# mkkellogg/GaussianSplats3D

Measured on NVIDIA H100. Metric: frames_per_sec, higher is better.
Workload: dtype int32 sort keys / f32 raster

## Files before the change

gaussiansplats3d_b200/csrc/raster_kernels.cuh:

```cuda
#pragma once
#include "common.cuh"
#include "sort_kernels.cuh"
#include "../../include/gsplat_b200.h"
#include <cuda_fp16.h>
#include "ellipse_mask.h"

namespace gs {

constexpr int kTile = 16;
constexpr int kTileShift = 4;
constexpr float kTransmittanceCutoff = 1.0f / 512.0f;

struct __align__(16) SplatRecord {
    float cx, cy;
    float g1x, g1y;
    float g2x, g2y;
    uint32_t hxhy;
    float a;
    float r, g, b;
    float ndc_z;
};

constexpr int kVisibleSlots = 64;
struct RasterControl {
// ... 83 lines not shown
        for (int r = 0; r < 4; ++r)
            o[4 * c + r] = a[r] * b[4 * c] + a[4 + r] * b[4 * c + 1] + a[8 + r] * b[4 * c + 2] + a[12 + r] * b[4 * c + 3];
}
__device__ inline void mat4_inverse_dev(const float *m, float *o) {
    float inv[16];
    inv[0] = m[5] * m[10] * m[15] - m[5] * m[11] * m[14] - m[9] * m[6] * m[15] + m[9] * m[7] * m[14] + m[13] * m[6] * m[11] - m[13] * m[7] * m[10];
    inv[4] = -m[4] * m[10] * m[15] + m[4] * m[11] * m[14] + m[8] * m[6] * m[15] - m[8] * m[7] * m[14] - m[12] * m[6] * m[11] + m[12] * m[7] * m[10];
    inv[8] = m[4] * m[9] * m[15] - m[4] * m[11] * m[13] - m[8] * m[5] * m[15] + m[8] * m[7] * m[13] + m[12] * m[5] * m[11] - m[12] * m[7] * m[9];
    inv[12] = -m[4] * m[9] * m[14] + m[4] * m[10] * m[13] + m[8] * m[5] * m[14] - m[8] * m[6] * m[13] - m[12] * m[5] * m[10] + m[12] * m[6] * m[9];
    inv[1] = -m[1] * m[10] * m[15] + m[1] * m[11] * m[14] + m[9] * m[2] * m[15] - m[9] * m[3] * m[14] - m[13] * m[2] * m[11] + m[13] * m[3] * m[10];
    inv[5] = m[0] * m[10] * m[15] - m[0] * m[11] * m[14] - m[8] * m[2] * m[15] + m[8] * m[3] * m[14] + m[12] * m[2] * m[11] - m[12] * m[3] * m[10];
    inv[9] = -m[0] * m[9] * m[15] + m[0] * m[11] * m[13] + m[8] * m[1] * m[15] - m[8] * m[3] * m[13] - m[12] * m[1] * m[11] + m[12] * m[3] * m[9];
    inv[13] = m[0] * m[9] * m[14] - m[0] * m[10] * m[13] - m[8] * m[1] * m[14] + m[8] * m[2] * m[13] + m[12] * m[1] * m[10] - m[12] * m[2] * m[9];
    inv[2] = m[1] * m[6] * m[15] - m[1] * m[7] * m[14] - m[5] * m[2] * m[15] + m[5] * m[3] * m[14] + m[13] * m[2] * m[7] - m[13] * m[3] * m[6];
    inv[6] = -m[0] * m[6] * m[15] + m[0] * m[7] * m[14] + m[4] * m[2] * m[15] - m[4] * m[3] * m[14] - m[12] * m[2] * m[7] + m[12] * m[3] * m[6];
    inv[10] = m[0] * m[5] * m[15] - m[0] * m[7] * m[13] - m[4] * m[1] * m[15] + m[4] * m[3] * m[13] + m[12] * m[1] * m[7] - m[12] * m[3] * m[5];
    inv[14] = -m[0] * m[5] * m[14] + m[0] * m[6] * m[13] + m[4] * m[1] * m[14] - m[4] * m[2] * m[13] - m[12] * m[1] * m[6] + m[12] * m[2] * m[5];
    inv[3] = -m[1] * m[6] * m[11] + m[1] * m[7] * m[10] + m[5] * m[2] * m[11] - m[5] * m[3] * m[10] - m[9] * m[2] * m[7] + m[9] * m[3] * m[6];
    inv[7] = m[0] * m[6] * m[11] - m[0] * m[7] * m[10] - m[4] * m[2] * m[11] + m[4] * m[3] * m[10] + m[8] * m[2] * m[7] - m[8] * m[3] * m[6];
    inv[11] = -m[0] * m[5] * m[11] + m[0] * m[7] * m[9] + m[4] * m[1] * m[11] - m[4] * m[3] * m[9] - m[8] * m[1] * m[7] + m[8] * m[3] * m[5];
    inv[15] = m[0] * m[5] * m[10] - m[0] * m[6] * m[9] - m[4] * m[1] * m[10] + m[4] * m[2] * m[9] + m[8] * m[1] * m[6] - m[8] * m[2] * m[5];
    const float det = m[0] * inv[0] + m[1] * inv[4] + m[2] * inv[8] + m[3] * inv[12];
    const float id = 1.0f / det;
#pragma unroll
    for (int i = 0; i < 16; ++i) o[i] = inv[i] * id;
}

constexpr int kProjThreads = 128;

template <bool COVF16, int SHFMT>
__global__ void __launch_bounds__(kProjThreads)
k_project(const uint4 *__restrict__ cc, const void *__restrict__ cov, const void *__restrict__ sh, int sh_data_degree,
          const uint32_t *__restrict__ scene_idx, const DynamicUniforms *__restrict__ dyn, const ProjParams *__restrict__ Pp, uint32_t count,
          SplatRecord *__restrict__ rec, ushort4 *__restrict__ rects, RasterControl *rctl) {
    pdl_enter();
    __shared__ ProjParams s_P;
    {
        const uint32_t *src = reinterpret_cast<const uint32_t *>(Pp);
        uint32_t *dst = reinterpret_cast<uint32_t *>(&s_P);
        for (int i = threadIdx.x; i < (int)(sizeof(ProjParams) / 4); i += kProjThreads) dst[i] = __ldg(src + i);
    }
    __syncthreads();
    const ProjParams &P = s_P;
    __shared__ float4 s_out[kProjThreads / 32][96];
    const uint32_t lane = threadIdx.x & 31;
    const uint32_t s = blockIdx.x * kProjThreads + threadIdx.x;
    uint32_t visible = 0;
    if (s < count) {
        SplatRecord o;
        o.cx = o.cy = o.g1x = o.g1y = o.g2x = o.g2y = o.a = o.r = o.g = o.b = 0.f;
        o.ndc_z = 2.0f;
        o.hxhy = 0;
        ushort4 rect = make_ushort4(1, 1, 0, 0);
        const int4 c4 = ld_nc_v4(cc + s);
        float V[6];
        if (COVF16) {
            const uint32_t *h32 = (const uint32_t *)cov + (size_t)s * 3;
#pragma unroll
            for (int k = 0; k < 3; ++k) {
                const uint32_t w = ld_nc_u32(h32 + k);
                const __half2 hh = *reinterpret_cast<const __half2 *>(&w);
                V[2 * k] = __low2float(hh); V[2 * k + 1] = __high2float(hh);
            }
        } else {
            const float2 *f2 = (const float2 *)cov + (size_t)s * 3;
            const float2 a0 = __ldg(f2), a1 = __ldg(f2 + 1), a2 = __ldg(f2 + 2);
            V[0] = a0.x; V[1] = a0.y; V[2] = a1.x; V[3] = a1.y; V[4] = a2.x; V[5] = a2.y;
// ... 139 lines not shown
                o.cy = (ndcy + 1.0f) * 0.5f * P.viewport[1];
                o.g1x = ex * is1; o.g1y = ey * is1;
                o.g2x = ey * is2; o.g2y = -ex * is2;
                o.ndc_z = ndcz; o.a = col[3];
                o.r = col[0]; o.g = col[1]; o.b = col[2];
                const bool in_depth = (ndcz >= -1.0f && ndcz <= 1.0f) && isfinite(s1) && isfinite(s2) && s1 > 0.f && s2 > 0.f;
                if (!in_depth && ndcz >= -1.0f && ndcz <= 1.0f) o.ndc_z = 2.0f;
                if (in_depth) {
                    const float b1x = ex * s1, b1y = ey * s1, b2x = ey * s2, b2y = -ex * s2;
                    const float hx = sqrtf(b1x * b1x + b2x * b2x) * 1.0005f + 0.01f;
                    const float hy = sqrtf(b1y * b1y + b2y * b2y) * 1.0005f + 0.01f;
                    const __half2 hh = __halves2half2(__float2half_ru(fminf(hx, 60000.f)), __float2half_ru(fminf(hy, 60000.f)));
                    o.hxhy = *reinterpret_cast<const uint32_t *>(&hh);
                    const float fx0 = ceilf(o.cx - hx - 0.5f), fx1 = floorf(o.cx + hx - 0.5f);
                    const float fy0 = ceilf(o.cy - hy - 0.5f), fy1 = floorf(o.cy + hy - 0.5f);
                    const float W1 = (float)(P.width - 1), H1 = (float)(P.height - 1);
                    if (fx1 >= 0.f && fy1 >= 0.f && fx0 <= W1 && fy0 <= H1 && fx0 <= fx1 && fy0 <= fy1) {
                        const int px0 = (int)fmaxf(fx0, 0.f), px1 = (int)fminf(fx1, W1);
                        const int py0 = (int)fmaxf(fy0, 0.f), py1 = (int)fminf(fy1, H1);
                        rect = make_ushort4((unsigned short)(px0 >> P.tile_shift), (unsigned short)(py0 >> P.tile_shift),
                                            (unsigned short)(px1 >> P.tile_shift), (unsigned short)(py1 >> P.tile_shift));
                        visible = 1;
                    }
                }
            }
        }
        float4 *stage = s_out[threadIdx.x >> 5];
        stage[lane * 3 + 0] = make_float4(o.cx, o.cy, o.g1x, o.g1y);
        stage[lane * 3 + 1] = make_float4(o.g2x, o.g2y, __uint_as_float(o.hxhy), o.a);
        stage[lane * 3 + 2] = make_float4(o.r, o.g, o.b, o.ndc_z);
        rects[s] = rect;
    }
    __syncwarp();
    {
        const uint32_t warp_first = blockIdx.x * kProjThreads + (threadIdx.x & ~31u);
        if (warp_first < count) {
            const uint32_t nrec = min(32u, count - warp_first);
            float4 *gdst = reinterpret_cast<float4 *>(rec + warp_first);
            const float4 *stage = s_out[threadIdx.x >> 5];
#pragma unroll
            for (int k = 0; k < 3; ++k) {
                const uint32_t idx = (uint32_t)k * 32 + lane;
                if (idx < nrec * 3) gdst[idx] = stage[idx];
            }
        }
    }
    const uint32_t nvis = __popc(__ballot_sync(0xffffffffu, visible));
    if ((threadIdx.x & 31) == 0 && nvis) atomicAdd(&rctl->visible_slots[((blockIdx.x * (kProjThreads / 32) + (threadIdx.x >> 5)) & (kVisibleSlots - 1)) * 8], nvis);
}

constexpr int kCoarseW = 8, kCoarseH = 4, kCoarseShiftX = 3, kCoarseShiftY = 2;
constexpr int kFinePerCoarse = kCoarseW * kCoarseH;

struct OwnMask { unsigned long long lo, hi; };
__host__ __device__ __forceinline__ bool own_diag(const OwnMask &m, int diag) {
    return ((diag < 64 ? m.lo >> diag : m.hi >> (diag - 64)) & 1ull) != 0ull;
}
__device__ __forceinline__ uint32_t own_count_range(const OwnMask &m, int d0, int d1) {
    uint32_t n = 0;
    if (d0 < 64) {
        const int hi = min(d1, 63);
        const unsigned long long w = (m.lo >> d0) & (hi - d0 == 63 ? ~0ull : ((1ull << (hi - d0 + 1)) - 1ull));
        n += __popcll(w);
    }
    if (d1 >= 64) {
        const int lo = max(d0, 64) - 64, hi = d1 - 64;
        const unsigned long long w = (m.hi >> lo) & (hi - lo == 63 ? ~0ull : ((1ull << (hi - lo + 1)) - 1ull));
        n += __popcll(w);
    }
    return n;
}
static inline OwnMask make_own_mask(uint32_t rank, uint32_t world) {
    OwnMask m{~0ull, ~0ull};
    if (world > 1) {
        m.lo = m.hi = 0;
        for (int d = 0; d < 128; ++d)
            if ((uint32_t)d % world == rank) { if (d < 64) m.lo |= 1ull << d; else m.hi |= 1ull << (d - 64); }
    }
    return m;
}
// ... 173 lines not shown

template <typename F>
__device__ __forceinline__ void round_instances(bool valid, uint32_t sid, ushort4 r, int coarse_x, const OwnMask &own, bool sharded, F f) {
    const int lane = threadIdx.x & 31;
    const bool nonempty = valid && r.z >= r.x && r.w >= r.y;
    const int cx0 = r.x >> kCoarseShiftX, cx1 = r.z >> kCoarseShiftX, cy0 = r.y >> kCoarseShiftY, cy1 = r.w >> kCoarseShiftY;
    const bool big = nonempty && (uint32_t)(cx1 - cx0 + 1) * (uint32_t)(cy1 - cy0 + 1) > 32u;
    if (nonempty && !big) {
#pragma unroll 1
        for (int cy = cy0; cy <= cy1; ++cy)
#pragma unroll 1
            for (int cx = cx0; cx <= cx1; ++cx) {
                if (sharded && !own_diag(own, cx + cy)) continue;
                f(lane, sid, cy * coarse_x + cx, fine_mask_in_coarse((int)r.x, (int)r.y, (int)r.z, (int)r.w, cx, cy));
            }
    }
    uint32_t multi = __ballot_sync(0xffffffffu, big);
    while (multi) {
        const int src = __ffs(multi) - 1;
        multi &= multi - 1;
        const uint32_t bsid = __shfl_sync(0xffffffffu, sid, src);
        const int bx0 = __shfl_sync(0xffffffffu, (int)r.x, src), by0 = __shfl_sync(0xffffffffu, (int)r.y, src);
        const int bx1 = __shfl_sync(0xffffffffu, (int)r.z, src), by1 = __shfl_sync(0xffffffffu, (int)r.w, src);
        const int ccx0 = bx0 >> kCoarseShiftX, ccy0 = by0 >> kCoarseShiftY;
        const int cw = (bx1 >> kCoarseShiftX) - ccx0 + 1, ntile = cw * ((by1 >> kCoarseShiftY) - ccy0 + 1);
        for (int i = lane; i < ntile; i += 32) {
            const int cy = ccy0 + i / cw, cx = ccx0 + i % cw;
            if (sharded && !own_diag(own, cx + cy)) continue;
            f(src, bsid, cy * coarse_x + cx, fine_mask_in_coarse(bx0, by0, bx1, by1, cx, cy));
        }
    }
}

__global__ void __launch_bounds__(kBinWarps * 32)
k_bin_count(const uint32_t *__restrict__ order, uint32_t render_count_host, const unsigned long long *__restrict__ n_dev, const ushort4 *__restrict__ rects,
            int coarse_x, uint32_t nt, uint32_t *__restrict__ hist, uint32_t stride, uint32_t *__restrict__ totals, ushort4 *__restrict__ rect_by_rank,
            OwnMask own, int sharded) {
    pdl_enter();
    constexpr int W = kBinWarps, ITEMS = kBinRankItems, NT = kBinTiles;
    const uint32_t n = n_dev ? (uint32_t)*n_dev : render_count_host;
    const uint32_t base = blockIdx.x * (uint32_t)(W * 32 * ITEMS);
    if (base >= n) return;
    __shared__ uint32_t s_hist[NT];
    for (uint32_t t = threadIdx.x; t < nt; t += W * 32) s_hist[t] = 0;
    __syncthreads();
    const int lane = threadIdx.x & 31, warp = threadIdx.x >> 5;
    const uint32_t run = base + (uint32_t)warp * (32 * ITEMS) + lane;
    uint32_t sid[ITEMS];
    ushort4 rc[ITEMS];
#pragma unroll
    for (int k = 0; k < ITEMS; ++k) {
        const uint32_t p = run + (uint32_t)k * 32;
        sid[k] = p < n ? ld_nc_u32(order + (n - 1u - p)) : 0xffffffffu;
    }
#pragma unroll
    for (int k = 0; k < ITEMS; ++k) rc[k] = sid[k] != 0xffffffffu ? rects[sid[k]] : make_ushort4(1, 1, 0, 0);
#pragma unroll
    for (int k = 0; k < ITEMS; ++k) {
        const uint32_t p = run + (uint32_t)k * 32;
        if (p < n) rect_by_rank[p] = rc[k];
    }
#pragma unroll 1
    for (int k = 0; k < ITEMS; ++k) {
        uint32_t id = 0; ushort4 r = make_ushort4(1, 1, 0, 0);
#pragma unroll
        for (int j = 0; j < ITEMS; ++j) if (j == k) { id = sid[j]; r = rc[j]; }
        round_instances(id != 0xffffffffu, id, r, coarse_x, own, sharded != 0, [&](int, uint32_t, int t, uint32_t) { atomicAdd(&s_hist[t], 1u); });
    }
    __syncthreads();
    for (uint32_t t = threadIdx.x; t < nt; t += W * 32) {
        const uint32_t v = s_hist[t];
        hist[(size_t)t * stride + blockIdx.x] = v;
        if (v) atomicAdd(&totals[t], v);
    }
}

__global__ void __launch_bounds__(1024)
k_bin_scan(uint32_t *__restrict__ hist, uint32_t stride, uint32_t ranks_per_chunk, uint32_t render_count_host, const unsigned long long *__restrict__ n_dev,
           const uint32_t *__restrict__ totals, uint32_t nt, uint2 *__restrict__ ranges, RasterControl *rctl, uint32_t *__restrict__ tile_order,
           unsigned long long capacity) {
    pdl_enter();
    __shared__ uint32_t s_scan[40];
    __shared__ uint32_t s_carry;
    {
        const uint32_t mine = totals[blockIdx.x];
        bool ahead = false;
        if (threadIdx.x < nt) { const uint32_t o = totals[threadIdx.x]; ahead = o > mine || (o == mine && threadIdx.x < blockIdx.x); }
        const int rank = __syncthreads_count(ahead);
        if (threadIdx.x == 0) tile_order[rank] = blockIdx.x;
    }
    const uint32_t n = n_dev ? (uint32_t)*n_dev : render_count_host;
    const uint32_t nchunks = (uint32_t)(((uint64_t)n + ranks_per_chunk - 1) / ranks_per_chunk);
    const uint32_t d = blockIdx.x;
    {
        uint32_t total;
        const uint32_t c = threadIdx.x < d ? totals[threadIdx.x] : 0u;
        (void)block_exclusive_scan<1024>(c, s_scan, total);
        if (threadIdx.x == 0) {
            s_carry = total;
            const uint32_t mine = totals[d];
            const unsigned long long lo = total, hi = lo + mine;
            ranges[d] = make_uint2((uint32_t)min(lo, capacity), (uint32_t)min(hi, capacity));
            if (d == nt - 1) rctl->total_instances = hi;
        }
    }
    __syncthreads();
    uint32_t *col = hist + (size_t)d * stride;
    for (uint32_t b = 0; b < nchunks; b += 1024) {
        const uint32_t t = b + threadIdx.x;
        const uint32_t v = t < nchunks ? col[t] : 0u;
        uint32_t total;
        const uint32_t ex = block_exclusive_scan<1024>(v, s_scan, total);
        const uint32_t carry = s_carry;
        if (t < nchunks) col[t] = ex + carry;
        __syncthreads();
        if (threadIdx.x == 0) s_carry = carry + total;
        __syncthreads();
    }
}

__global__ void __launch_bounds__(kBinWarps * 32)
k_bin_place(const uint32_t *__restrict__ order, uint32_t render_count_host, const unsigned long long *__restrict__ n_dev, const ushort4 *__restrict__ rect_by_rank,
            int coarse_x, uint32_t nt, const uint32_t *__restrict__ offsets, uint32_t stride, unsigned long long *__restrict__ list, unsigned long long capacity,
            RasterControl *rctl, OwnMask own, int sharded, int pack_ok) {
    pdl_enter();
    constexpr int W = kBinWarps, ITEMS = kBinRankItems, NT = kBinTiles;
    const uint32_t n = n_dev ? (uint32_t)*n_dev : render_count_host;
    const uint32_t base = blockIdx.x * (uint32_t)(W * 32 * ITEMS);
    if (base >= n) return;
    __shared__ uint32_t s_pre[W][NT];
    __shared__ __align__(8) uint32_t s_mask[W][NT];
    static_assert(NT * 4 >= 32 * ITEMS * 8, "the mask row of a warp doubles as the staging buffer of its compacted items");
    for (uint32_t i = threadIdx.x; i < (uint32_t)(W * NT); i += W * 32) (&s_pre[0][0])[i] = 0;
    __syncthreads();
    const int lane = threadIdx.x & 31, warp = threadIdx.x >> 5;
    const uint32_t run = base + (uint32_t)warp * (32 * ITEMS) + lane;
    uint32_t sid[ITEMS];
    ushort4 rc[ITEMS];
#pragma unroll
    for (int k = 0; k < ITEMS; ++k) {
        const uint32_t p = run + (uint32_t)k * 32;
        sid[k] = p < n ? ld_nc_u32(order + (n - 1u - p)) : 0xffffffffu;
        rc[k] = p < n ? rect_by_rank[p] : make_ushort4(1, 1, 0, 0);
    }
    uint32_t *my_pre = s_pre[warp], *my_mask = s_mask[warp];
    uint32_t nvalid = 32u * ITEMS;
    if (pack_ok) {
        const uint32_t lt = lanemask_lt();
        unsigned long long *stage = reinterpret_cast<unsigned long long *>(my_mask);
        uint32_t before = 0;
#pragma unroll
        for (int k = 0; k < ITEMS; ++k) {
            const bool keep = sid[k] != 0xffffffffu && (sharded ? rect_touches_owned(rc[k], own) : (rc[k].z >= rc[k].x && rc[k].w >= rc[k].y));
            const uint32_t bal = __ballot_sync(0xffffffffu, keep);
            if (keep) stage[before + __popc(bal & lt)] = ((unsigned long long)((uint32_t)rc[k].x | ((uint32_t)rc[k].y << 8) | ((uint32_t)rc[k].z << 16) | ((uint32_t)rc[k].w << 24)) << 32) | sid[k];
            before += __popc(bal);
        }
        nvalid = before;
        __syncwarp();
#pragma unroll
        for (int k = 0; k < ITEMS; ++k) {
            const uint32_t j = (uint32_t)k * 32u + (uint32_t)lane;
            sid[k] = 0xffffffffu;
            rc[k] = make_ushort4(1, 1, 0, 0);
            if (j < nvalid) {
                const unsigned long long v = stage[j];
                const uint32_t pr = (uint32_t)(v >> 32);
                sid[k] = (uint32_t)v;
                rc[k] = make_ushort4((unsigned short)(pr & 255u), (unsigned short)((pr >> 8) & 255u), (unsigned short)((pr >> 16) & 255u), (unsigned short)(pr >> 24));
            }
        }
        __syncwarp();
#pragma unroll
        for (int i = 0; i < NT / 32; ++i) my_mask[i * 32 + lane] = 0u;
        __syncwarp();
    }
#pragma unroll
    for (int k = 0; k < ITEMS; ++k)
        if ((uint32_t)k * 32u < nvalid)
            round_instances(sid[k] != 0xffffffffu, sid[k], rc[k], coarse_x, own, sharded != 0, [&](int, uint32_t, int t, uint32_t) { atomicAdd(&my_pre[t], 1u); });
    __syncthreads();
    for (uint32_t t = threadIdx.x; t < nt; t += W * 32) {
        uint32_t at = offsets[(size_t)t * stride + blockIdx.x];
#pragma unroll
        for (int w = 0; w < W; ++w) {
            const uint32_t c = s_pre[w][t];
            s_pre[w][t] = at;
            at += c;
        }
    }
    __syncthreads();
    bool overflow = false;
#pragma unroll
    for (int k = 0; k < ITEMS; ++k) {
        if ((uint32_t)k * 32u >= nvalid) break;
        const bool valid = sid[k] != 0xffffffffu;
#pragma unroll
        for (int i = 0; i < NT / 32; ++i) my_mask[i * 32 + lane] = 0u;
        __syncwarp();
        round_instances(valid, sid[k], rc[k], coarse_x, own, sharded != 0, [&](int owner, uint32_t, int t, uint32_t) {
            atomicOr(&my_mask[t], 1u << owner);
            atomicAdd(&my_pre[t], 1u);
        });
        __syncwarp();
        round_instances(valid, sid[k], rc[k], coarse_x, own, sharded != 0, [&](int owner, uint32_t sid_o, int t, uint32_t fmask) {
            const uint32_t m = my_mask[t];
            const unsigned long long at = (unsigned long long)(my_pre[t] - (uint32_t)__popc(m)) + __popc(m & ((1u << owner) - 1u));
            if (at < capacity) list[at] = ((unsigned long long)fmask << 32) | sid_o;
            else overflow = true;
        });
        __syncwarp();
    }
    if (overflow) rctl->overflow = 1;
}

__global__ void __launch_bounds__(kBinThreads)
// ... 296 lines not shown
    size_t n = 0;
    cudaError_t ensure(size_t count) {
        if (count <= n) return cudaSuccess;
        if (p) cudaFree(p);
        p = nullptr; n = 0;
        cudaError_t e = cudaMalloc((void **)&p, (count ? count : 1) * sizeof(T));
        if (e == cudaSuccess) n = count;
        return e;
    }
    void release() { if (p) cudaFree(p); p = nullptr; n = 0; }
};

struct RasterState {
    RBuf<uint4> cc;
    RBuf<unsigned char> cov, sh;
    RBuf<uint32_t> scene_idx;
    int cov_format = GS_COV_F32, sh_format = GS_SH_NONE;
    uint32_t sh_degree = 0, uploaded = 0;
    bool have_scene_idx = false;
    RBuf<SplatRecord> records;
    RBuf<ushort4> rects;
    RBuf<uint32_t> block_sums;
    RBuf<uint32_t> warp_sums;
    RBuf<uint32_t> super_sums;
    uint32_t super_stride = 0;
    RBuf<uint16_t> ikeys[2];
    RBuf<unsigned long long> ivals[2];
    RBuf<unsigned long long> list;
    RBuf<uint2> ranges;
    RBuf<RasterControl> rctl;
    RBuf<SortControl> sctl;
    RBuf<uint32_t> tile_hist;
    RBuf<uint32_t> bin_hist;
    RBuf<ushort4> rect_by_rank;
    RBuf<uint32_t> tile_order;
    RBuf<uint32_t> bin_totals;
    uint32_t bin_stride = 0;
    RBuf<DynamicUniforms> dyn;
    RBuf<ProjParams> projp;
    RBuf<unsigned char> frame;
    RBuf<unsigned char> frame_alt;
    unsigned char *frame_half2 = nullptr;
    size_t frame_half_bytes = 0;
    int frame_parity = 0;
    uint32_t *snap_base = nullptr;
    uint32_t snap_stride = 0;
    const uint32_t *snap_sort_ctl = nullptr;
    bool snapshot_taken = false;
    RBuf<gs_projected_splat> exported;
    RBuf<PeerSync> peer_sync_local;
    PeerSync *peer_sync = nullptr;
    void *peer_frame = nullptr;
    bool peer_root = false, peer_attached = false;
    unsigned long long instance_capacity = 0;
    uint32_t hist_stride = 0;
    int sm_count = 132;
    int last_format = GS_FRAME_RGBA32F;
    size_t last_frame_bytes = 0;
};

#define RCU(call)                                                                                                 \
    do {                                                                                                          \
        cudaError_t _e = (call);                                                                                  \
        if (_e != cudaSuccess) { snprintf(raster_err(), 512, "%s -> %s (%s:%d)", #call, cudaGetErrorString(_e), __FILE__, __LINE__); return GS_ERR_CUDA; } \
    } while (0)

static inline char *raster_err() { return g_gs_err; }

static inline int frame_tile_shift(uint32_t width, uint32_t height) {
    const uint32_t cx = (width + kTile * kCoarseW - 1) / (kTile * kCoarseW), cy = (height + kTile * kCoarseH - 1) / (kTile * kCoarseH);
    return (cx * cy <= (uint32_t)kBinTiles) ? kTileShift : kTileShift + 1;
}

static inline uint32_t frame_coarse_tiles(uint32_t width, uint32_t height) {
    const uint32_t tpx = 1u << frame_tile_shift(width, height);
    const uint32_t tiles_x = (width + tpx - 1) / tpx, tiles_y = (height + tpx - 1) / tpx;
    return ((tiles_x + kCoarseW - 1) / kCoarseW) * ((tiles_y + kCoarseH - 1) / kCoarseH);
}

static int raster_init(RasterState &rs, const gs_config &c, int sm_count) {
    rs.sm_count = sm_count;
    const size_t n = c.max_splat_count ? c.max_splat_count : 1;
    RCU(rs.rctl.ensure(1));
    RCU(cudaMemset(rs.rctl.p, 0, sizeof(RasterControl)));
    RCU(rs.sctl.ensure(1));
    RCU(rs.dyn.ensure(2));
    RCU(rs.projp.ensure(2));
    RCU(cudaMemset(rs.dyn.p, 0, 2 * sizeof(DynamicUniforms)));
    if (c.max_width && c.max_height) {
        RCU(rs.cc.ensure(n));
        RCU(rs.records.ensure(n));
        RCU(rs.rects.ensure(n));
        RCU(rs.block_sums.ensure((n + kBinTile - 1) / kBinTile + 1));
        RCU(rs.warp_sums.ensure(((n + kBinTile - 1) / kBinTile + 1) * (kBinThreads / 32)));
        rs.super_stride = (uint32_t)(((n + kBinTile - 1) / kBinTile) / kBinThreads + 2);
        RCU(rs.super_sums.ensure(2 * (size_t)rs.super_stride));
        const char *f = getenv("GS_INSTANCE_FACTOR");
        const double factor = f ? atof(f) : 4.0;
        const size_t tiles = (size_t)((c.max_width + kTile - 1) / kTile) * ((c.max_height + kTile - 1) / kTile);
        rs.instance_capacity = (unsigned long long)(factor * (double)n) + 4ull * tiles + 65536ull;
        if (rs.instance_capacity > 0xfffffff0ull) rs.instance_capacity = 0xfffffff0ull;
        RCU(rs.list.ensure(rs.instance_capacity));
        RCU(rs.ranges.ensure(65536));
        RCU(rs.tile_order.ensure(65536));
        RCU(rs.frame.ensure((size_t)c.max_width * (c.max_height + kTile) * 16));
        if (frame_coarse_tiles(c.max_width, c.max_height) > (uint32_t)kBinTiles) {
            for (int i = 0; i < 2; ++i) { RCU(rs.ikeys[i].ensure(rs.instance_capacity)); RCU(rs.ivals[i].ensure(rs.instance_capacity)); }
            RCU(rs.tile_hist.ensure(radix_tile_hist_words(rs.instance_capacity, 2, &rs.hist_stride)));
        }
        {
            const size_t coarse = (size_t)((c.max_width + kTile * kCoarseW - 1) / (kTile * kCoarseW)) * ((c.max_height + kTile * kCoarseH - 1) / (kTile * kCoarseH));
            const size_t chunks = (n + kBinRanks - 1) / kBinRanks + 1;
            rs.bin_stride = (uint32_t)((chunks + 31) & ~(size_t)31);
            RCU(rs.bin_hist.ensure(std::max<size_t>(coarse, 1) * rs.bin_stride));
            RCU(rs.rect_by_rank.ensure(n));
            RCU(rs.bin_totals.ensure(kBinTiles));
            RCU(cudaMemset(rs.bin_totals.p, 0, kBinTiles * 4));
        }
    }
    return GS_OK;
}

static void raster_release(RasterState &rs) {
    rs.cc.release(); rs.cov.release(); rs.sh.release(); rs.scene_idx.release(); rs.records.release(); rs.rects.release();
    rs.block_sums.release(); rs.warp_sums.release(); rs.super_sums.release(); rs.ikeys[0].release(); rs.ikeys[1].release(); rs.ivals[0].release(); rs.ivals[1].release();
    rs.list.release(); rs.ranges.release(); rs.rctl.release(); rs.sctl.release(); rs.tile_hist.release(); rs.bin_hist.release(); rs.bin_totals.release(); rs.rect_by_rank.release(); rs.tile_order.release();
    rs.dyn.release(); rs.projp.release(); rs.frame.release(); rs.frame_alt.release(); rs.peer_sync_local.release(); rs.exported.release();
}

static int raster_upload(RasterState &rs, const gs_config &c, const gs_splat_data &d, cudaStream_t st) {
    if (!c.max_width || !c.max_height) { snprintf(raster_err(), 512, "engine created without a framebuffer (max_width/max_height = 0)"); return GS_ERR_NOT_READY; }
    if ((uint64_t)d.from + d.count > c.max_splat_count) { snprintf(raster_err(), 512, "splat data [%u,%u) exceeds max_splat_count %u", d.from, d.from + d.count, c.max_splat_count); return GS_ERR_CAPACITY; }
    if (!d.centers_colors || !d.covariances) { snprintf(raster_err(), 512, "gs_upload_splat_data: null centers_colors/covariances"); return GS_ERR_BAD_ARG; }
    if (d.sh_degree > 2) { snprintf(raster_err(), 512, "sh_degree %u > 2", d.sh_degree); return GS_ERR_BAD_ARG; }
    const size_t n = c.max_splat_count;
    const size_t cov_elt = d.cov_format == GS_COV_F16 ? 12 : 24;
    const size_t ncomp = d.sh_degree == 2 ? 24 : (d.sh_degree == 1 ? 9 : 0);
    const size_t sh_elt = ncomp * (d.sh_format == GS_SH_F16 ? 2 : (d.sh_format == GS_SH_U8 ? 1 : 4));
    if (d.from == 0) rs.uploaded = 0;
    if (rs.uploaded && (rs.cov_format != d.cov_format || (rs.sh_degree != d.sh_degree) || (ncomp && rs.sh_format != d.sh_format))) {
        snprintf(raster_err(), 512, "splat data format changed between partial uploads"); return GS_ERR_BAD_ARG;
    }
    rs.cov_format = d.cov_format;
    rs.sh_degree = d.sh_degree;
    rs.sh_format = ncomp ? d.sh_format : GS_SH_NONE;
    RCU(rs.cov.ensure(n * cov_elt + 16));
    if (ncomp) {
        if (!d.spherical_harmonics) { snprintf(raster_err(), 512, "sh_degree %u without spherical_harmonics", d.sh_degree); return GS_ERR_BAD_ARG; }
        RCU(rs.sh.ensure(n * sh_elt + 16));
    }
    RCU(cudaMemcpyAsync(rs.cc.p + d.from, d.centers_colors, (size_t)d.count * 16, cudaMemcpyHostToDevice, st));
    RCU(cudaMemcpyAsync(rs.cov.p + (size_t)d.from * cov_elt, d.covariances, (size_t)d.count * cov_elt, cudaMemcpyHostToDevice, st));
    if (ncomp) RCU(cudaMemcpyAsync(rs.sh.p + (size_t)d.from * sh_elt, d.spherical_harmonics, (size_t)d.count * sh_elt, cudaMemcpyHostToDevice, st));
    if (d.scene_indexes) {
        RCU(rs.scene_idx.ensure(n));
        RCU(cudaMemcpyAsync(rs.scene_idx.p + d.from, d.scene_indexes, (size_t)d.count * 4, cudaMemcpyHostToDevice, st));
        rs.have_scene_idx = true;
    }
    rs.uploaded = std::max<uint32_t>(rs.uploaded, d.from + d.count);
    return GS_OK;
}

static unsigned char *raster_second_frame(RasterState &rs) { return rs.frame_alt.p ? rs.frame_alt.p : rs.frame_half2; }
static void *raster_frame_ptr(RasterState &rs, int) { return (rs.frame_parity && raster_second_frame(rs)) ? raster_second_frame(rs) : rs.frame.p; }

template <bool COVF16>
static void launch_project(RasterState &rs, uint32_t count, cudaStream_t st) {
    const int blocks = (int)((count + kProjThreads - 1) / kProjThreads);
    const uint32_t *sc = rs.have_scene_idx ? rs.scene_idx.p : nullptr;
#define GS_PROJ(FMT) gs_launch(k_project<COVF16, FMT>, blocks, kProjThreads, 0, st, rs.cc.p, rs.cov.p, rs.sh.p, (int)rs.sh_degree, sc, rs.dyn.p + rs.frame_parity, rs.projp.p + rs.frame_parity, count, rs.records.p, rs.rects.p, rs.rctl.p)
    switch (rs.sh_format) {
        case GS_SH_F16: GS_PROJ(GS_SH_F16); break;
        case GS_SH_U8: GS_PROJ(GS_SH_U8); break;
        case GS_SH_F32: GS_PROJ(GS_SH_F32); break;
        default: GS_PROJ(GS_SH_NONE); break;
    }
#undef GS_PROJ
}

static int raster_upload_params(RasterState &rs, const gs_config &c, const gs_uniforms &u, const gs_render_params &p, cudaStream_t st) {
    const int tshift = frame_tile_shift(p.width, p.height), tpx = 1 << tshift;
    const int tiles_x = (p.width + tpx - 1) / tpx, tiles_y = (p.height + tpx - 1) / tpx;
    const uint32_t world = c.world_size, rank = c.rank;
    ProjParams P{};
    memcpy(P.mv, u.model_view, 64); memcpy(P.proj, u.projection, 64);
    memcpy(P.cam, u.camera_position, 12);
    P.focal[0] = u.focal[0]; P.focal[1] = u.focal[1]; P.viewport[0] = u.viewport[0]; P.viewport[1] = u.viewport[1];
    P.inv_focal_adj = u.inverse_focal_adjustment; P.ortho_zoom = u.ortho_zoom; P.orthographic = u.orthographic_mode;
    P.splat_scale = u.splat_scale; P.point_cloud = u.point_cloud_mode; P.sh_degree = u.sh_degree; P.antialiased = u.antialiased;
    P.kernel2d = u.kernel_2d_size; P.max_size = u.max_screen_space_splat_size; P.fade_in_complete = u.fade_in_complete;
    memcpy(P.scene_center, u.scene_center, 12); P.fade_start = u.visible_region_fade_start_radius;
    P.dynamic = u.dynamic_mode; P.optional_effects = u.enable_optional_effects; P.scene_count = (int)u.scene_count;
    P.tiles_x = tiles_x; P.tiles_y = tiles_y; P.rank = rank; P.world = world; P.width = (int)p.width; P.height = (int)p.height;
    P.tile_shift = tshift;
    RCU(cudaMemcpyAsync(rs.projp.p + rs.frame_parity, &P, sizeof(P), cudaMemcpyHostToDevice, st));
    if (u.dynamic_mode || u.enable_optional_effects || rs.sh_format == GS_SH_U8) {
        DynamicUniforms du;
        memcpy(du.view, u.view_matrix, 64);
        memcpy(du.transforms, u.scene_transforms, sizeof(du.transforms));
        memcpy(du.sh8_min, u.sh8_min, sizeof(du.sh8_min)); memcpy(du.sh8_max, u.sh8_max, sizeof(du.sh8_max));
        memcpy(du.opacity, u.scene_opacity, sizeof(du.opacity)); memcpy(du.visibility, u.scene_visibility, sizeof(du.visibility));
        RCU(cudaMemcpyAsync(rs.dyn.p + rs.frame_parity, &du, sizeof(du), cudaMemcpyHostToDevice, st));
    }
// ... 10 lines not shown
    }
    if (p.render_count > rs.uploaded) { snprintf(raster_err(), 512, "render_count %u > uploaded splats %u", p.render_count, rs.uploaded); return GS_ERR_CAPACITY; }
    const int tshift = frame_tile_shift(p.width, p.height), tpx = 1 << tshift;
    const int tiles_x = (p.width + tpx - 1) / tpx, tiles_y = (p.height + tpx - 1) / tpx;
    const uint32_t world = c.world_size, rank = c.rank;
    const uint32_t local_tiles = (uint32_t)tiles_x * (uint32_t)tiles_y;
    uint32_t launches = 0;

    if (upload_params) { int prc = raster_upload_params(rs, c, u, p, st); if (prc) return prc; }
    const int coarse_x = (tiles_x + kCoarseW - 1) / kCoarseW, coarse_y = (tiles_y + kCoarseH - 1) / kCoarseH;
    const uint32_t ncoarse = (uint32_t)coarse_x * (uint32_t)coarse_y;
    if (ncoarse > 65536u) { snprintf(raster_err(), 512, "frame %ux%u needs %u coarse tiles (> 65536)", p.width, p.height, ncoarse); return GS_ERR_BAD_ARG; }
    int tile_bits = 1;
    while ((1u << tile_bits) < std::max(ncoarse, 2u)) ++tile_bits;
    const PassPlan pl = make_plan_bits(tile_bits);
    if (phases & 1) {
        gs_launch(k_raster_init, 8, 256, 0, st, rs.rctl.p, rs.sctl.p, rs.ranges.p, ncoarse, rs.super_sums.p, 2 * rs.super_stride, rs.bin_totals.p, rs.tile_order.p);
        ++launches;
        prof.mark("k_raster_init", st);
        if (world > 1 && rs.peer_root) { k_peer_release<<<1, 1, 0, st>>>(rs.peer_sync, rs.rctl.p, (uint32_t)(rs.frame_parity && rs.frame_half2)); ++launches; }
        const uint32_t count = rs.uploaded;
        if (rs.cov_format == GS_COV_F16) launch_project<true>(rs, count, st); else launch_project<false>(rs, count, st);
        ++launches;
        prof.mark("k_project", st);
        if (record_events) RCU(cudaEventRecord(ev_project, st));
    }
    if (!(phases & 2)) { tm.kernel_launches = launches; return GS_OK; }
    rs.snapshot_taken = false;
    const bool counting_sort = ncoarse <= (uint32_t)kBinTiles;
    if (p.render_count && local_tiles && counting_sort) {
        const OwnMask own = make_own_mask(rank, world);
        const int sharded = world > 1 ? 1 : 0;
        const uint32_t chunks = (p.render_count + kBinRanks - 1u) / kBinRanks;
        gs_launch(k_bin_count, chunks, kBinWarps * 32, 0, st, d_order, p.render_count, order_count_dev, rs.rects.p, coarse_x, ncoarse, rs.bin_hist.p, rs.bin_stride,
                  rs.bin_totals.p, rs.rect_by_rank.p, own, sharded);
        ++launches;
        prof.mark("k_bin_count", st);
        gs_launch(k_bin_scan, ncoarse, 1024, 0, st, rs.bin_hist.p, rs.bin_stride, (uint32_t)kBinRanks, p.render_count, order_count_dev, rs.bin_totals.p, ncoarse, rs.ranges.p, rs.rctl.p, rs.tile_order.p, rs.instance_capacity);
        ++launches;
        prof.mark("k_bin_scan", st);
        gs_launch(k_bin_place, chunks, kBinWarps * 32, 0, st, d_order, p.render_count, order_count_dev, rs.rect_by_rank.p, coarse_x, ncoarse, rs.bin_hist.p, rs.bin_stride,
                  rs.list.p, rs.instance_capacity, rs.rctl.p, own, sharded, (tiles_x <= 256 && tiles_y <= 256) ? 1 : 0);
        ++launches;
        prof.mark("k_bin_place", st);
    }
    if (p.render_count && local_tiles && !counting_sort) {
        const uint32_t chunks = (p.render_count + kBinTile - 1) / kBinTile;
        gs_launch(k_tile_count, chunks, kBinThreads, 0, st, d_order, p.render_count, order_count_dev, rs.rects.p, rs.block_sums.p, rs.warp_sums.p, rs.super_sums.p, make_own_mask(rank, world), world > 1 ? 1 : 0);
        ++launches;
        prof.mark("k_tile_count", st);
        gs_launch(k_tile_emit, chunks, kBinThreads, 0, st, d_order, p.render_count, order_count_dev, rs.rects.p, rs.block_sums.p, rs.warp_sums.p, rs.super_sums.p, coarse_x, rs.ikeys[0].p,
                                                    rs.ivals[0].p, rs.instance_capacity, rs.rctl.p, make_own_mask(rank, world), world > 1 ? 1 : 0);
        ++launches;
        prof.mark("k_tile_emit", st);
        static const RadixNames names = {{"k_radix_hist[tile,0]", "k_radix_hist[tile,1]", "k_radix_hist[tile,2]", "k_radix_hist[tile,3]"},
                                         {"k_radix_scan[tile,0]", "k_radix_scan[tile,1]", "k_radix_scan[tile,2]", "k_radix_scan[tile,3]"},
                                         {"k_radix_scatter[tile,0]", "k_radix_scatter[tile,1]", "k_radix_scatter[tile,2]", "k_radix_scatter[tile,3]"}};
        const unsigned long long *n_dev = &rs.rctl.p->total_instances;
        radix_sort_pairs<uint16_t, unsigned long long>(rs.ikeys[0].p, rs.ikeys[1].p, rs.ivals[0].p, 0u, kValArray, rs.ivals[1].p, rs.ivals[0].p, rs.list.p, 0u,
                                                       n_dev, rs.instance_capacity, pl, rs.sctl.p, rs.tile_hist.p, rs.hist_stride, false, rs.ranges.p, st, launches,
                                                       &prof, names);
    }
    if (record_events) RCU(cudaEventRecord(ev_bin, st));
    if (local_tiles) {
        const bool peer_mode = world > 1 && (rs.peer_root || rs.peer_attached);
        void *target = raster_frame_ptr(rs, p.frame_format);
        if (world > 1 && !peer_mode) RCU(cudaMemsetAsync(target, 0, (size_t)p.width * p.height * (p.frame_format == GS_FRAME_RGBA8 ? 4 : 16), st));
        if (peer_mode && rs.peer_attached) {
            k_peer_wait_release<<<1, 1, 0, st>>>(rs.peer_sync, rs.rctl.p);
            ++launches;
            target = rs.peer_frame;
        }
        const uint32_t grid = ncoarse * kFinePerCoarse;
        const bool to_peer = peer_mode && rs.peer_attached;
        const StatusSnapshot snap{rs.snap_sort_ctl, reinterpret_cast<const uint32_t *>(rs.rctl.p),
// ... 43 lines not shown
```

Before: 3261.

## Compact visible splats in bin count and reuse packed items in bin place

The projection kernel now writes a per-warp visibility bitmask. The bin-count kernel uses that mask to skip rect loads for culled splats when the rect array would not fit in L2. It then block-compacts the kept (rect, id) pairs into packed items written to global memory, and balances the histogram work across warps. The bin-place kernel reads the compacted items and per-block counts instead of re-reading the order array and rects, and exits early for empty blocks. This adds an item buffer and more shared memory in bin count, which can lower occupancy.

Result: no change. 3234 (median of 6 runs) (-0.8%).

```diff
diff --git a/gaussiansplats3d_b200/csrc/raster_kernels.cuh b/gaussiansplats3d_b200/csrc/raster_kernels.cuh
--- a/gaussiansplats3d_b200/csrc/raster_kernels.cuh
+++ b/gaussiansplats3d_b200/csrc/raster_kernels.cuh
@@ -139,7 +139,7 @@
 __global__ void __launch_bounds__(kProjThreads)
 k_project(const uint4 *__restrict__ cc, const void *__restrict__ cov, const void *__restrict__ sh, int sh_data_degree,
           const uint32_t *__restrict__ scene_idx, const DynamicUniforms *__restrict__ dyn, const ProjParams *__restrict__ Pp, uint32_t count,
-          SplatRecord *__restrict__ rec, ushort4 *__restrict__ rects, RasterControl *rctl) {
+          SplatRecord *__restrict__ rec, ushort4 *__restrict__ rects, uint32_t *__restrict__ vis_bits, RasterControl *rctl) {
     pdl_enter();
     __shared__ ProjParams s_P;
     {
@@ -345,8 +345,8 @@
         rects[s] = rect;
     }
     __syncwarp();
+    const uint32_t warp_first = blockIdx.x * kProjThreads + (threadIdx.x & ~31u);
     {
-        const uint32_t warp_first = blockIdx.x * kProjThreads + (threadIdx.x & ~31u);
         if (warp_first < count) {
             const uint32_t nrec = min(32u, count - warp_first);
             float4 *gdst = reinterpret_cast<float4 *>(rec + warp_first);
@@ -358,7 +358,9 @@
             }
         }
     }
-    const uint32_t nvis = __popc(__ballot_sync(0xffffffffu, visible));
+    const uint32_t vis_mask = __ballot_sync(0xffffffffu, visible);
+    if (lane == 0 && warp_first < count) vis_bits[warp_first >> 5] = vis_mask;
+    const uint32_t nvis = __popc(vis_mask);
     if ((threadIdx.x & 31) == 0 && nvis) atomicAdd(&rctl->visible_slots[((blockIdx.x * (kProjThreads / 32) + (threadIdx.x >> 5)) & (kVisibleSlots - 1)) * 8], nvis);
 }
 
@@ -598,42 +600,90 @@
     }
 }
 
-__global__ void __launch_bounds__(kBinWarps * 32)
-k_bin_count(const uint32_t *__restrict__ order, uint32_t render_count_host, const unsigned long long *__restrict__ n_dev, const ushort4 *__restrict__ rects,
-            int coarse_x, uint32_t nt, uint32_t *__restrict__ hist, uint32_t stride, uint32_t *__restrict__ totals, ushort4 *__restrict__ rect_by_rank,
-            OwnMask own, int sharded) {
+template <bool PACK> struct BinItem;
+template <> struct BinItem<true> {
+    using T = unsigned long long;
+    static __device__ __forceinline__ T make(ushort4 r, uint32_t sid) {
+        return ((unsigned long long)((uint32_t)r.x | ((uint32_t)r.y << 8) | ((uint32_t)r.z << 16) | ((uint32_t)r.w << 24)) << 32) | sid;
+    }
+    static __device__ __forceinline__ void get(T v, ushort4 &r, uint32_t &sid) {
+        const uint32_t pr = (uint32_t)(v >> 32);
+        sid = (uint32_t)v;
+        r = make_ushort4((unsigned short)(pr & 255u), (unsigned short)((pr >> 8) & 255u), (unsigned short)((pr >> 16) & 255u), (unsigned short)(pr >> 24));
+    }
+};
+template <> struct BinItem<false> {
+    using T = uint4;
+    static __device__ __forceinline__ T make(ushort4 r, uint32_t sid) {
+        return make_uint4((uint32_t)r.x | ((uint32_t)r.y << 16), (uint32_t)r.z | ((uint32_t)r.w << 16), sid, 0u);
+    }
+    static __device__ __forceinline__ void get(T v, ushort4 &r, uint32_t &sid) {
+        sid = v.z;
+        r = make_ushort4((unsigned short)(v.x & 0xffffu), (unsigned short)(v.x >> 16), (unsigned short)(v.y & 0xffffu), (unsigned short)(v.y >> 16));
+    }
+};
+
+template <bool PACK, bool BITS>
+__global__ void __launch_bounds__(kBinWarps * 32, 3)
+k_bin_count(const uint32_t *__restrict__ order, uint32_t render_count_host, const unsigned long long *__restrict__ n_dev, const uint32_t *__restrict__ vis_bits,
+            const ushort4 *__restrict__ rects, int coarse_x, uint32_t nt, uint32_t *__restrict__ hist, uint32_t stride, uint32_t *__restrict__ totals,
+            typename BinItem<PACK>::T *__restrict__ items, uint32_t *__restrict__ kept, OwnMask own, int sharded) {
     pdl_enter();
     constexpr int W = kBinWarps, ITEMS = kBinRankItems, NT = kBinTiles;
     const uint32_t n = n_dev ? (uint32_t)*n_dev : render_count_host;
     const uint32_t base = blockIdx.x * (uint32_t)(W * 32 * ITEMS);
     if (base >= n) return;
     __shared__ uint32_t s_hist[NT];
+    __shared__ uint32_t s_warp[W];
+    __shared__ typename BinItem<PACK>::T s_items[W * 32 * ITEMS];
     for (uint32_t t = threadIdx.x; t < nt; t += W * 32) s_hist[t] = 0;
-    __syncthreads();
     const int lane = threadIdx.x & 31, warp = threadIdx.x >> 5;
     const uint32_t run = base + (uint32_t)warp * (32 * ITEMS) + lane;
-    uint32_t sid[ITEMS];
+    uint32_t sid[ITEMS], bal[ITEMS];
     ushort4 rc[ITEMS];
 #pragma unroll
     for (int k = 0; k < ITEMS; ++k) {
         const uint32_t p = run + (uint32_t)k * 32;
         sid[k] = p < n ? ld_nc_u32(order + (n - 1u - p)) : 0xffffffffu;
     }
-#pragma unroll
-    for (int k = 0; k < ITEMS; ++k) rc[k] = sid[k] != 0xffffffffu ? rects[sid[k]] : make_ushort4(1, 1, 0, 0);
+    bool keep[ITEMS];
+#pragma unroll
+    for (int k = 0; k < ITEMS; ++k) keep[k] = sid[k] != 0xffffffffu && (!BITS || ((vis_bits[sid[k] >> 5] >> (sid[k] & 31u)) & 1u));
+#pragma unroll
+    for (int k = 0; k < ITEMS; ++k) rc[k] = keep[k] ? rects[sid[k]] : make_ushort4(1, 1, 0, 0);
+    uint32_t mine = 0;
 #pragma unroll
     for (int k = 0; k < ITEMS; ++k) {
-        const uint32_t p = run + (uint32_t)k * 32;
-        if (p < n) rect_by_rank[p] = rc[k];
-    }
+        if (sharded) keep[k] = keep[k] && rect_touches_owned(rc[k], own);
+        else if (!BITS) keep[k] = keep[k] && rc[k].z >= rc[k].x && rc[k].w >= rc[k].y;
+        bal[k] = __ballot_sync(0xffffffffu, keep[k]);
+        mine += __popc(bal[k]);
+    }
+    if (lane == 0) s_warp[warp] = mine;
+    __syncthreads();
+    uint32_t at = 0, total = 0;
+#pragma unroll
+    for (int w = 0; w < W; ++w) { const uint32_t c = s_warp[w]; at += w < warp ? c : 0u; total += c; }
+    const uint32_t lt = lanemask_lt();
+#pragma unroll
+    for (int k = 0; k < ITEMS; ++k) {
+        if ((bal[k] >> lane) & 1u) s_items[at + __popc(bal[k] & lt)] = BinItem<PACK>::make(rc[k], sid[k]);
+        at += __popc(bal[k]);
+    }
+    __syncthreads();
+    for (uint32_t j = threadIdx.x; j < total; j += W * 32) items[base + j] = s_items[j];
+    const uint32_t per_warp = (total + W * 32 - 1) / (W * 32) * 32;
+    const uint32_t first = (uint32_t)warp * per_warp;
+    const uint32_t nvalid = first < total ? min(per_warp, total - first) : 0u;
 #pragma unroll 1
-    for (int k = 0; k < ITEMS; ++k) {
-        uint32_t id = 0; ushort4 r = make_ushort4(1, 1, 0, 0);
-#pragma unroll
-        for (int j = 0; j < ITEMS; ++j) if (j == k) { id = sid[j]; r = rc[j]; }
+    for (uint32_t j0 = 0; j0 < nvalid; j0 += 32) {
+        uint32_t id = 0xffffffffu;
+        ushort4 r = make_ushort4(1, 1, 0, 0);
+        if (j0 + lane < nvalid) BinItem<PACK>::get(s_items[first + j0 + lane], r, id);
         round_instances(id != 0xffffffffu, id, r, coarse_x, own, sharded != 0, [&](int, uint32_t, int t, uint32_t) { atomicAdd(&s_hist[t], 1u); });
     }
     __syncthreads();
+    if (threadIdx.x == 0) kept[blockIdx.x] = total;
     for (uint32_t t = threadIdx.x; t < nt; t += W * 32) {
         const uint32_t v = s_hist[t];
         hist[(size_t)t * stride + blockIdx.x] = v;
@@ -685,69 +735,46 @@
     }
 }
 
+template <bool PACK>
 __global__ void __launch_bounds__(kBinWarps * 32)
-k_bin_place(const uint32_t *__restrict__ order, uint32_t render_count_host, const unsigned long long *__restrict__ n_dev, const ushort4 *__restrict__ rect_by_rank,
-            int coarse_x, uint32_t nt, const uint32_t *__restrict__ offsets, uint32_t stride, unsigned long long *__restrict__ list, unsigned long long capacity,
-            RasterControl *rctl, OwnMask own, int sharded, int pack_ok) {
+k_bin_place(uint32_t render_count_host, const unsigned long long *__restrict__ n_dev, const typename BinItem<PACK>::T *__restrict__ items,
+            const uint32_t *__restrict__ kept, int coarse_x, uint32_t nt, const uint32_t *__restrict__ offsets, uint32_t stride,
+            unsigned long long *__restrict__ list, unsigned long long capacity, RasterControl *rctl, OwnMask own, int sharded) {
     pdl_enter();
     constexpr int W = kBinWarps, ITEMS = kBinRankItems, NT = kBinTiles;
     const uint32_t n = n_dev ? (uint32_t)*n_dev : render_count_host;
     const uint32_t base = blockIdx.x * (uint32_t)(W * 32 * ITEMS);
     if (base >= n) return;
+    const uint32_t nkept = kept[blockIdx.x];
+    if (nkept == 0) return;
     __shared__ uint32_t s_pre[W][NT];
-    __shared__ __align__(8) uint32_t s_mask[W][NT];
-    static_assert(NT * 4 >= 32 * ITEMS * 8, "the mask row of a warp doubles as the staging buffer of its compacted items");
+    __shared__ uint32_t s_mask[W][NT];
+    static_assert(NT <= W * 32, "one tile per thread in the offset prefix");
+    const uint32_t my_off = threadIdx.x < nt ? offsets[(size_t)threadIdx.x * stride + blockIdx.x] : 0u;
     for (uint32_t i = threadIdx.x; i < (uint32_t)(W * NT); i += W * 32) (&s_pre[0][0])[i] = 0;
     __syncthreads();
     const int lane = threadIdx.x & 31, warp = threadIdx.x >> 5;
-    const uint32_t run = base + (uint32_t)warp * (32 * ITEMS) + lane;
+    const uint32_t per_warp = (nkept + W * 32 - 1) / (W * 32) * 32;
+    const uint32_t first = (uint32_t)warp * per_warp;
+    const uint32_t nvalid = first < nkept ? min(per_warp, nkept - first) : 0u;
     uint32_t sid[ITEMS];
     ushort4 rc[ITEMS];
 #pragma unroll
     for (int k = 0; k < ITEMS; ++k) {
-        const uint32_t p = run + (uint32_t)k * 32;
-        sid[k] = p < n ? ld_nc_u32(order + (n - 1u - p)) : 0xffffffffu;
-        rc[k] = p < n ? rect_by_rank[p] : make_ushort4(1, 1, 0, 0);
+        const uint32_t j = (uint32_t)k * 32u + (uint32_t)lane;
+        sid[k] = 0xffffffffu;
+        rc[k] = make_ushort4(1, 1, 0, 0);
+        if (j < nvalid) BinItem<PACK>::get(items[base + first + j], rc[k], sid[k]);
     }
     uint32_t *my_pre = s_pre[warp], *my_mask = s_mask[warp];
-    uint32_t nvalid = 32u * ITEMS;
-    if (pack_ok) {
-        const uint32_t lt = lanemask_lt();
-        unsigned long long *stage = reinterpret_cast<unsigned long long *>(my_mask);
-        uint32_t before = 0;
-#pragma unroll
-        for (int k = 0; k < ITEMS; ++k) {
-            const bool keep = sid[k] != 0xffffffffu && (sharded ? rect_touches_owned(rc[k], own) : (rc[k].z >= rc[k].x && rc[k].w >= rc[k].y));
-            const uint32_t bal = __ballot_sync(0xffffffffu, keep);
-            if (keep) stage[before + __popc(bal & lt)] = ((unsigned long long)((uint32_t)rc[k].x | ((uint32_t)rc[k].y << 8) | ((uint32_t)rc[k].z << 16) | ((uint32_t)rc[k].w << 24)) << 32) | sid[k];
-            before += __popc(bal);
-        }
-        nvalid = before;
-        __syncwarp();
-#pragma unroll
-        for (int k = 0; k < ITEMS; ++k) {
-            const uint32_t j = (uint32_t)k * 32u + (uint32_t)lane;
-            sid[k] = 0xffffffffu;
-            rc[k] = make_ushort4(1, 1, 0, 0);
-            if (j < nvalid) {
-                const unsigned long long v = stage[j];
-                const uint32_t pr = (uint32_t)(v >> 32);
-                sid[k] = (uint32_t)v;
-                rc[k] = make_ushort4((unsigned short)(pr & 255u), (unsigned short)((pr >> 8) & 255u), (unsigned short)((pr >> 16) & 255u), (unsigned short)(pr >> 24));
-            }
-        }
-        __syncwarp();
-#pragma unroll
-        for (int i = 0; i < NT / 32; ++i) my_mask[i * 32 + lane] = 0u;
-        __syncwarp();
-    }
 #pragma unroll
     for (int k = 0; k < ITEMS; ++k)
         if ((uint32_t)k * 32u < nvalid)
             round_instances(sid[k] != 0xffffffffu, sid[k], rc[k], coarse_x, own, sharded != 0, [&](int, uint32_t, int t, uint32_t) { atomicAdd(&my_pre[t], 1u); });
     __syncthreads();
-    for (uint32_t t = threadIdx.x; t < nt; t += W * 32) {
-        uint32_t at = offsets[(size_t)t * stride + blockIdx.x];
+    if (threadIdx.x < nt) {
+        const uint32_t t = threadIdx.x;
+        uint32_t at = my_off;
 #pragma unroll
         for (int w = 0; w < W; ++w) {
             const uint32_t c = s_pre[w][t];
@@ -1110,7 +1137,10 @@
     RBuf<SortControl> sctl;
     RBuf<uint32_t> tile_hist;
     RBuf<uint32_t> bin_hist;
-    RBuf<ushort4> rect_by_rank;
+    RBuf<uint32_t> vis_bits;
+    RBuf<uint4> bin_items;
+    bool bin_items_wide = false;
+    RBuf<uint32_t> bin_kept;
     RBuf<uint32_t> tile_order;
     RBuf<uint32_t> bin_totals;
     uint32_t bin_stride = 0;
@@ -1133,6 +1163,7 @@
     unsigned long long instance_capacity = 0;
     uint32_t hist_stride = 0;
     int sm_count = 132;
+    size_t l2_bytes = 50u << 20;
     int last_format = GS_FRAME_RGBA32F;
     size_t last_frame_bytes = 0;
 };
@@ -1158,6 +1189,12 @@
 
 static int raster_init(RasterState &rs, const gs_config &c, int sm_count) {
     rs.sm_count = sm_count;
+    {
+        int dev = 0, l2 = 0;
+        RCU(cudaGetDevice(&dev));
+        RCU(cudaDeviceGetAttribute(&l2, cudaDevAttrL2CacheSize, dev));
+        rs.l2_bytes = (size_t)l2;
+    }
     const size_t n = c.max_splat_count ? c.max_splat_count : 1;
     RCU(rs.rctl.ensure(1));
     RCU(cudaMemset(rs.rctl.p, 0, sizeof(RasterControl)));
@@ -1169,6 +1206,7 @@
         RCU(rs.cc.ensure(n));
         RCU(rs.records.ensure(n));
         RCU(rs.rects.ensure(n));
+        RCU(rs.vis_bits.ensure((n + 31) / 32));
         RCU(rs.block_sums.ensure((n + kBinTile - 1) / kBinTile + 1));
         RCU(rs.warp_sums.ensure(((n + kBinTile - 1) / kBinTile + 1) * (kBinThreads / 32)));
         rs.super_stride = (uint32_t)(((n + kBinTile - 1) / kBinTile) / kBinThreads + 2);
@@ -1191,7 +1229,9 @@
             const size_t chunks = (n + kBinRanks - 1) / kBinRanks + 1;
             rs.bin_stride = (uint32_t)((chunks + 31) & ~(size_t)31);
             RCU(rs.bin_hist.ensure(std::max<size_t>(coarse, 1) * rs.bin_stride));
-            RCU(rs.rect_by_rank.ensure(n));
+            rs.bin_items_wide = c.max_width > 256u * kTile || c.max_height > 256u * kTile;
+            RCU(rs.bin_items.ensure(rs.bin_items_wide ? n : (n + 1) / 2));
+            RCU(rs.bin_kept.ensure(chunks));
             RCU(rs.bin_totals.ensure(kBinTiles));
             RCU(cudaMemset(rs.bin_totals.p, 0, kBinTiles * 4));
         }
@@ -1202,7 +1242,8 @@
 static void raster_release(RasterState &rs) {
     rs.cc.release(); rs.cov.release(); rs.sh.release(); rs.scene_idx.release(); rs.records.release(); rs.rects.release();
     rs.block_sums.release(); rs.warp_sums.release(); rs.super_sums.release(); rs.ikeys[0].release(); rs.ikeys[1].release(); rs.ivals[0].release(); rs.ivals[1].release();
-    rs.list.release(); rs.ranges.release(); rs.rctl.release(); rs.sctl.release(); rs.tile_hist.release(); rs.bin_hist.release(); rs.bin_totals.release(); rs.rect_by_rank.release(); rs.tile_order.release();
+    rs.list.release(); rs.ranges.release(); rs.rctl.release(); rs.sctl.release(); rs.tile_hist.release(); rs.bin_hist.release(); rs.bin_totals.release(); rs.tile_order.release();
+    rs.vis_bits.release(); rs.bin_items.release(); rs.bin_kept.release();
     rs.dyn.release(); rs.projp.release(); rs.frame.release(); rs.frame_alt.release(); rs.peer_sync_local.release(); rs.exported.release();
 }
 
@@ -1246,7 +1287,7 @@
 static void launch_project(RasterState &rs, uint32_t count, cudaStream_t st) {
     const int blocks = (int)((count + kProjThreads - 1) / kProjThreads);
     const uint32_t *sc = rs.have_scene_idx ? rs.scene_idx.p : nullptr;
-#define GS_PROJ(FMT) gs_launch(k_project<COVF16, FMT>, blocks, kProjThreads, 0, st, rs.cc.p, rs.cov.p, rs.sh.p, (int)rs.sh_degree, sc, rs.dyn.p + rs.frame_parity, rs.projp.p + rs.frame_parity, count, rs.records.p, rs.rects.p, rs.rctl.p)
+#define GS_PROJ(FMT) gs_launch(k_project<COVF16, FMT>, blocks, kProjThreads, 0, st, rs.cc.p, rs.cov.p, rs.sh.p, (int)rs.sh_degree, sc, rs.dyn.p + rs.frame_parity, rs.projp.p + rs.frame_parity, count, rs.records.p, rs.rects.p, rs.vis_bits.p, rs.rctl.p)
     switch (rs.sh_format) {
         case GS_SH_F16: GS_PROJ(GS_SH_F16); break;
         case GS_SH_U8: GS_PROJ(GS_SH_U8); break;
@@ -1323,15 +1364,25 @@
         const OwnMask own = make_own_mask(rank, world);
         const int sharded = world > 1 ? 1 : 0;
         const uint32_t chunks = (p.render_count + kBinRanks - 1u) / kBinRanks;
-        gs_launch(k_bin_count, chunks, kBinWarps * 32, 0, st, d_order, p.render_count, order_count_dev, rs.rects.p, coarse_x, ncoarse, rs.bin_hist.p, rs.bin_stride,
-                  rs.bin_totals.p, rs.rect_by_rank.p, own, sharded);
+        const bool pack = tiles_x <= 256 && tiles_y <= 256;
+        if (!pack && !rs.bin_items_wide) { snprintf(raster_err(), 512, "frame %ux%u: binning item buffer sized for 8-byte items", p.width, p.height); return GS_ERR_BAD_ARG; }
+        unsigned long long *items8 = reinterpret_cast<unsigned long long *>(rs.bin_items.p);
+        const bool bits = (size_t)rs.uploaded * sizeof(ushort4) > rs.l2_bytes / 2;
+#define GS_BIN_COUNT(PACK, BITS, ITEMS) gs_launch(k_bin_count<PACK, BITS>, chunks, kBinWarps * 32, 0, st, d_order, p.render_count, order_count_dev, \
+                                                  rs.vis_bits.p, rs.rects.p, coarse_x, ncoarse, rs.bin_hist.p, rs.bin_stride, rs.bin_totals.p, ITEMS, \
+                                                  rs.bin_kept.p, own, sharded)
+        if (pack) { if (bits) GS_BIN_COUNT(true, true, items8); else GS_BIN_COUNT(true, false, items8); }
+        else { if (bits) GS_BIN_COUNT(false, true, rs.bin_items.p); else GS_BIN_COUNT(false, false, rs.bin_items.p); }
+#undef GS_BIN_COUNT
         ++launches;
         prof.mark("k_bin_count", st);
         gs_launch(k_bin_scan, ncoarse, 1024, 0, st, rs.bin_hist.p, rs.bin_stride, (uint32_t)kBinRanks, p.render_count, order_count_dev, rs.bin_totals.p, ncoarse, rs.ranges.p, rs.rctl.p, rs.tile_order.p, rs.instance_capacity);
         ++launches;
         prof.mark("k_bin_scan", st);
-        gs_launch(k_bin_place, chunks, kBinWarps * 32, 0, st, d_order, p.render_count, order_count_dev, rs.rect_by_rank.p, coarse_x, ncoarse, rs.bin_hist.p, rs.bin_stride,
-                  rs.list.p, rs.instance_capacity, rs.rctl.p, own, sharded, (tiles_x <= 256 && tiles_y <= 256) ? 1 : 0);
+        if (pack) gs_launch(k_bin_place<true>, chunks, kBinWarps * 32, 0, st, p.render_count, order_count_dev, items8, rs.bin_kept.p, coarse_x, ncoarse,
+                            rs.bin_hist.p, rs.bin_stride, rs.list.p, rs.instance_capacity, rs.rctl.p, own, sharded);
+        else gs_launch(k_bin_place<false>, chunks, kBinWarps * 32, 0, st, p.render_count, order_count_dev, rs.bin_items.p, rs.bin_kept.p, coarse_x, ncoarse,
+                       rs.bin_hist.p, rs.bin_stride, rs.list.p, rs.instance_capacity, rs.rctl.p, own, sharded);
         ++launches;
         prof.mark("k_bin_place", st);
     }
```
